# dropbox/rust-brotli

Measured on AMD Instinct MI355X. Metric: compress MB/s at q5 lgwin22, higher is better.
Workload: dtype u8; 1 GPU; 64 MiB synthetic English-like text per GPU, quality=5, lgwin=22, one-shot BrotliEncoderCompress (H6), input and stream resident in HBM; input_bytes_total=67108864, compressed_bytes=16370400

## Files before the change

### rust-brotli_amd/csrc/lz77_kernels.hip

```cpp
#include <hip/hip_runtime.h>
#include <stdexcept>
#include <string>
#include <utility>
#include <string.h>
#include <mutex>
#include <vector>

#include "device_api.h"
#include "lz77_chain.h"
#include "lz77_rows.h"
#include "lz77_groups.h"
#include "device_scan.h"
#include "lz77_parse_args.h"
#include "zopfli_device.h"
#include "batch_greedy_device.h"

namespace brotli_mi355x {

void hip_check(hipError_t e, const char* what) {
  if (e == hipSuccess) return;
  (void)hipGetLastError();
  throw std::runtime_error(std::string("HIP error in ") + what + ": " + hipGetErrorString(e));
}

__global__ __launch_bounds__(256) void k_compute_keys(const uint8_t* __restrict__ text, uint16_t* __restrict__ keys,
                                                      uint32_t n, uint32_t valid_n, uint32_t kind, uint32_t bucket_bits,
                                                      uint64_t hash_mask, uint32_t* __restrict__ run_samples,
                                                      const uint16_t* __restrict__ dict_hash, uint32_t* __restrict__ dict_items) {
  uint32_t i = blockIdx.x * blockDim.x + threadIdx.x;
  const uint32_t stride = gridDim.x * blockDim.x;
  for (; i < n; i += stride) {
    if (dict_items != nullptr) {
      const uint32_t h = ((br_load32(text + i) * 0x1e35a7bdu) >> (32 - 14)) << 1;
      dict_items[i] = (uint32_t)dict_hash[h] | ((uint32_t)dict_hash[h + 1] << 16);
    }
    uint32_t key = 0xffffu;
    if (i < valid_n) {
      if ((i & 63u) == 0 && i + 16 <= n) {
        const uint64_t v = br_load64(text + i);
        if (v == (v & 0xffull) * 0x0101010101010101ull && br_load64(text + i + 8) == v && *(volatile uint32_t*)run_samples < 4096u)
          atomicAdd(run_samples, 1u);
      }
      if (kind == 6) {
        const uint64_t v = (br_load64(text + i) & hash_mask) * 0x1fe35a7bd3579bd3ull;
        key = (uint32_t)(v >> (64 - bucket_bits));
      } else {
        const uint32_t v = br_load32(text + i) * 0x1e35a7bdu;
        key = v >> (32 - bucket_bits);
      }
    }
    keys[i] = (uint16_t)key;
  }
  if (dict_items != nullptr && blockIdx.x == 0 && threadIdx.x == 0) {
    const uint32_t h = ((br_load32(text + n) * 0x1e35a7bdu) >> (32 - 14)) << 1;
    dict_items[n] = (uint32_t)dict_hash[h] | ((uint32_t)dict_hash[h + 1] << 16);
  }
}

void lz77_compute_keys(const Lz77Params& P, const Lz77Buffers& B) {
  const uint32_t n = P.total_bytes;
  const uint32_t valid_n = n >= P.htl ? n - P.htl + 1 : 0;
  const uint64_t hash_mask = P.hasher_kind == 6 ? (0xffffffffffffffffull >> (64 - 8 * P.hash_len)) : 0;
  if (n == 0) return;
  uint32_t blocks = (n + 255) / 256;
  if (blocks > 8192) blocks = 8192;
  dev_memset(B.changed_count + 8, 0, 4);
  hipLaunchKernelGGL(k_compute_keys, dim3(blocks), dim3(256), 0, BR_STREAM, B.text, B.keys, n, valid_n, P.hasher_kind, P.bucket_bits,
                     hash_mask, B.changed_count + 8, dev_tables().dict_hash, B.dict_items);
  HIP_CHECK(hipGetLastError());
}

__global__ __launch_bounds__(64) void k_init_flag_tails(const Segment* __restrict__ segments, uint32_t num_segments, uint32_t htl,
                                                         uint8_t* __restrict__ flags) {
  const uint32_t k = blockIdx.x * blockDim.x + threadIdx.x;
  if (k >= num_segments) return;
  const Segment g = segments[k];
  if (!(g.flags & kSegFirstInBlock)) return;
  const uint32_t bs = g.blk_start, be = g.blk_end;
  if (g.block_index == 0 && be - bs >= htl - 1 && bs >= 3) flags[bs - 3] = flags[bs - 2] = flags[bs - 1] = 1;
  const uint32_t store_end = (be - bs >= htl) ? be - htl + 1 : bs;
  for (uint32_t q = store_end; q < be; ++q) flags[q] = (q + 3 >= be && (g.flags & kSegTailStitched)) ? 1 : 0;
}

void lz77_init_flags(const Lz77Params& P, const Lz77Buffers& B, uint32_t first_block_start, const uint8_t* prefix_flags_host,
                     uint32_t prefix_flags_bytes) {
  const uint32_t M = P.total_bytes, P0 = P.prefix_bytes, htl = P.htl;
  dev_memset(B.flags[0], 0, (size_t)M + 64);
  if (P0 > htl - 1) HIP_CHECK(hipMemsetAsync(B.flags[0], 1, P0 - (htl - 1), BR_STREAM));
  if (prefix_flags_host && prefix_flags_bytes) {
    HIP_CHECK(hipMemcpyAsync(B.flags[0], prefix_flags_host, prefix_flags_bytes, hipMemcpyHostToDevice, BR_STREAM));
  }
  if (M > first_block_start) HIP_CHECK(hipMemsetAsync(B.flags[0] + first_block_start, 1, M - first_block_start, BR_STREAM));
  if (P.num_segments) {
    hipLaunchKernelGGL(k_init_flag_tails, dim3((P.num_segments + 63) / 64), dim3(64), 0, BR_STREAM, B.segments, P.num_segments, htl, B.flags[0]);
  }
  HIP_CHECK(hipMemcpyAsync(B.flags[1], B.flags[0], (size_t)M + 64, hipMemcpyDeviceToDevice, BR_STREAM));
  HIP_CHECK(hipGetLastError());
}

static constexpr uint32_t kSortTile = 4096;

__global__ __launch_bounds__(256) void k_radix_hist(const uint16_t* __restrict__ keys, uint32_t n, uint32_t shift,
                                                     uint32_t num_tiles, uint32_t* __restrict__ hist) {
  __shared__ uint32_t h[256];
  h[threadIdx.x] = 0;
  __syncthreads();
  const uint32_t base = blockIdx.x * kSortTile;
  for (uint32_t r = 0; r < 16; ++r) {
    const uint32_t i = base + r * 256 + threadIdx.x;
    if (i < n) atomicAdd(&h[(keys[i] >> shift) & 255u], 1u);
  }
  __syncthreads();
  hist[threadIdx.x * num_tiles + blockIdx.x] = h[threadIdx.x];
}

__global__ __launch_bounds__(256) void k_radix_scatter(const uint16_t* __restrict__ keys_in, const uint32_t* __restrict__ vals_in,
                                                        uint16_t* __restrict__ keys_out, uint32_t* __restrict__ vals_out, uint32_t n,
                                                        uint32_t shift, uint32_t num_tiles, const uint32_t* __restrict__ offsets,
                                                        const uint8_t* __restrict__ text, const uint16_t* __restrict__ tags_in,
                                                        uint16_t* __restrict__ tags_out) {
  __shared__ uint32_t gbase[256];
  __shared__ uint32_t lstart[256];
  __shared__ uint32_t run[256];
  __shared__ uint32_t wcount[4][256];
  __shared__ uint32_t wave_total[4];
  __shared__ uint16_t skey[kSortTile];
  __shared__ uint32_t sval[kSortTile];
  __shared__ uint16_t stagv[kSortTile];
  const int tid = threadIdx.x, lane = tid & 63, w = tid >> 6;
  const uint32_t tile_base = blockIdx.x * kSortTile;
  const uint32_t tile_n = n - tile_base < kSortTile ? n - tile_base : kSortTile;
  {
    const uint32_t idx = (uint32_t)tid * num_tiles + blockIdx.x;
    const uint32_t here = offsets[idx];
    const uint32_t next = idx + 1 < 256u * num_tiles ? offsets[idx + 1] : n;
    const uint32_t count = next - here;
    gbase[tid] = here;
    uint32_t incl = count;
    for (uint32_t off = 1; off < 64; off <<= 1) {
      const uint32_t up = (uint32_t)__shfl_up((int)incl, off, 64);
      if ((uint32_t)lane >= off) incl += up;
    }
    if (lane == 63) wave_total[w] = incl;
    __syncthreads();
    uint32_t before = 0;
    for (int i = 0; i < w; ++i) before += wave_total[i];
    lstart[tid] = before + incl - count;
    run[tid] = before + incl - count;
  }
  __syncthreads();
  for (uint32_t r = 0; r < 16; ++r) {
    const uint32_t i = tile_base + r * 256 + tid;
    const bool valid = i < n;
    uint32_t key = 0, val = 0, d = 0, tag = 0;
    if (valid) {
      key = keys_in[i];
      val = vals_in ? vals_in[i] : i;
      d = (key >> shift) & 255u;
      if (tags_out) tag = tags_in ? tags_in[i] : br_tag16(br_load32(text + val));
    }
#pragma unroll
    for (int j = 0; j < 4; ++j) wcount[w][lane * 4 + j] = 0;
    __syncthreads();
    unsigned long long peers = __ballot(valid);
#pragma unroll
    for (int bit = 0; bit < 8; ++bit) {
      const bool one = (d >> bit) & 1u;
      const unsigned long long b = __ballot(one);
      peers &= one ? b : ~b;
    }
    const uint32_t rank_in_wave = __popcll(peers & ((1ull << lane) - 1ull));
    if (valid && rank_in_wave == 0) wcount[w][d] = __popcll(peers);
    __syncthreads();
    if (valid) {
      uint32_t at = run[d] + rank_in_wave;
      for (int i2 = 0; i2 < w; ++i2) at += wcount[i2][d];
      skey[at] = (uint16_t)key;
      sval[at] = val;
      if (tags_out) stagv[at] = (uint16_t)tag;
    }
    __syncthreads();
    run[tid] += wcount[0][tid] + wcount[1][tid] + wcount[2][tid] + wcount[3][tid];
    __syncthreads();
  }
  for (uint32_t at = tid; at < tile_n; at += 256) {
    const uint32_t key = skey[at];
    const uint32_t d = (key >> shift) & 255u;
    const uint32_t dst = gbase[d] + (at - lstart[d]);
    keys_out[dst] = (uint16_t)key;
    vals_out[dst] = sval[at];
    if (tags_out) tags_out[dst] = stagv[at];
  }
}

size_t lz77_sort_tmp_bytes(uint32_t total_bytes) {
  const size_t n = total_bytes;
  const size_t tiles = (n + kSortTile - 1) / kSortTile + 1;
  return n * 10 + 2048 + tiles * 256 * 4 + (tiles * 256 / kScanTile + 1024) * 8 + (n / kScanTile + 1024) * 8 + 4096;
}

void lz77_key_ranges(const Lz77Params& P, const Lz77Buffers& B);

void lz77_sort_by_key(const Lz77Params& P, const Lz77Buffers& B) {
  const uint32_t n = P.total_bytes;
  if (n == 0) return;
  const uint32_t tiles = (n + kSortTile - 1) / kSortTile;
  uint8_t* tmp = (uint8_t*)B.sort_tmp;
  uint16_t* keys_tmp = (uint16_t*)tmp;
  tmp += ((size_t)n * 2 + 255) & ~(size_t)255;
  uint32_t* vals_tmp = (uint32_t*)tmp;
  tmp += ((size_t)n * 4 + 255) & ~(size_t)255;
  uint16_t* tags_tmp = (uint16_t*)tmp;
  tmp += ((size_t)n * 2 + 255) & ~(size_t)255;
  uint32_t* hist = (uint32_t*)tmp;
  tmp += (size_t)tiles * 256 * 4;
  uint32_t* scratch = (uint32_t*)tmp;
  hipLaunchKernelGGL(k_radix_hist, dim3(tiles), dim3(256), 0, BR_STREAM, B.keys, n, 0u, tiles, hist);
  exclusive_scan_u32(hist, tiles * 256, scratch);
  hipLaunchKernelGGL(k_radix_scatter, dim3(tiles), dim3(256), 0, BR_STREAM, B.keys, (const uint32_t*)nullptr, keys_tmp, vals_tmp, n, 0u, tiles,
                     hist, (const uint8_t*)B.text, (const uint16_t*)nullptr, B.stag ? tags_tmp : (uint16_t*)nullptr);
  hipLaunchKernelGGL(k_radix_hist, dim3(tiles), dim3(256), 0, BR_STREAM, keys_tmp, n, 8u, tiles, hist);
  exclusive_scan_u32(hist, tiles * 256, scratch);
  hipLaunchKernelGGL(k_radix_scatter, dim3(tiles), dim3(256), 0, BR_STREAM, keys_tmp, vals_tmp, B.sorted_keys, B.by_key, n, 8u, tiles, hist,
                     (const uint8_t*)B.text, (const uint16_t*)tags_tmp, B.stag);
  HIP_CHECK(hipGetLastError());
  lz77_key_ranges(P, B);
}

__global__ __launch_bounds__(256) void k_key_ranges(const uint16_t* __restrict__ sorted_keys, uint32_t n, uint32_t* __restrict__ key_first,
                                                     uint32_t* __restrict__ key_last) {
  const uint32_t i = blockIdx.x * blockDim.x + threadIdx.x;
  if (i >= n) return;
  const uint16_t k = sorted_keys[i];
  if (i == 0 || sorted_keys[i - 1] != k) key_first[k] = i;
  if (i + 1 == n || sorted_keys[i + 1] != k) key_last[k] = i + 1;
}

struct InitialFlagGeometry {
  uint32_t enabled, first_block_start, prefix_bytes, block_bytes, total_bytes, prefix_stored_end;
};

__global__ __launch_bounds__(256) void k_rank_gather(const uint32_t* __restrict__ by_key, const uint8_t* __restrict__ flags, uint32_t n,
                                                      uint8_t* __restrict__ fbits, uint32_t* __restrict__ tile_sums,
                                                      InitialFlagGeometry ig, uint32_t masked_bits) {
  __shared__ uint32_t wave_sum[4];
  const uint32_t base = blockIdx.x * kScanTile + threadIdx.x * 4;
  uint32_t local = 0, packed = 0;
#pragma unroll
  for (int j = 0; j < 4; ++j)
    if (base + j < n) {
      const uint32_t p = by_key[base + j];
      uint32_t f;
      bool known = false;
      if (ig.enabled) {
        if (p >= ig.first_block_start) {
          known = ((p - ig.prefix_bytes) % ig.block_bytes) + 16 < ig.block_bytes && p + 16 < ig.total_bytes;
        } else {
          known = p + 16 < ig.prefix_stored_end;
        }
      }
      const uint32_t fl = known ? 1u : (uint32_t)flags[p];
      f = fl & 1u;
      packed |= (f | ((masked_bits && (fl & kFlagMasked)) ? kSlotMasked : 0u)) << (8 * j);
      local += f;
    }
  if (base < n) *(uint32_t*)(fbits + base) = packed;
  for (int off = 32; off > 0; off >>= 1) local += __shfl_down(local, off, 64);
  if ((threadIdx.x & 63) == 0) wave_sum[threadIdx.x >> 6] = local;
  __syncthreads();
  if (threadIdx.x == 0) tile_sums[blockIdx.x] = wave_sum[0] + wave_sum[1] + wave_sum[2] + wave_sum[3];
}

__global__ __launch_bounds__(256) void k_key_bases(const uint8_t* __restrict__ fbits, const uint32_t* __restrict__ tile_offsets,
                                                    const uint32_t* __restrict__ key_first, const uint32_t* __restrict__ key_last,
                                                    uint32_t* __restrict__ key_base) {
  const uint32_t k = blockIdx.x * blockDim.x + threadIdx.x;
  if (k >= 65536) return;
  const uint32_t i0 = key_first[k];
  if (key_last[k] <= i0) return;
  const uint32_t tile = i0 / kScanTile;
  uint32_t g = tile_offsets[tile];
  uint32_t i = tile * kScanTile;
  for (; i + 4 <= i0; i += 4) g += (*(const uint32_t*)(fbits + i) * 0x01010101u) >> 24;
  for (; i < i0; ++i) g += fbits[i];
  key_base[k] = g;
}

__device__ __forceinline__ uint32_t ring_count_at(uint32_t p, uint32_t local_rank, uint32_t key, const uint32_t* count_base, uint32_t reset_pos,
                                                  const uint32_t* reset_counts);
__device__ __forceinline__ uint32_t ring_count(uint32_t local_rank, uint32_t base) {
  const uint32_t num = (local_rank + base) & 0xffffu;
  return num < local_rank ? num : local_rank;
}

__device__ __forceinline__ uint32_t ring_count_at(uint32_t p, uint32_t local_rank, uint32_t key, const uint32_t* count_base, uint32_t reset_pos,
                                                  const uint32_t* reset_counts) {
  if (reset_pos != 0 && p >= reset_pos) {
    const uint32_t since = local_rank - reset_counts[key];
    return since & 0xffffu;
  }
  return ring_count(local_rank, count_base ? count_base[key] : 0u);
}

__global__ __launch_bounds__(256) void k_rank_apply(const uint32_t* __restrict__ by_key, const uint16_t* __restrict__ sorted_keys,
                                                     const uint8_t* __restrict__ fbits, uint32_t n, const uint32_t* __restrict__ tile_offsets,
                                                     const uint32_t* __restrict__ key_first, const uint32_t* __restrict__ key_base,
                                                     uint32_t* __restrict__ sorted, uint2* __restrict__ info,
                                                     const uint32_t* __restrict__ count_base, uint32_t reset_pos,
                                                     const uint32_t* __restrict__ reset_counts, const uint16_t* __restrict__ stag,
                                                     uint16_t* __restrict__ sorted_tag, const uint8_t* __restrict__ flags_if_masked) {
  __shared__ uint32_t wave_sum[4];
  const uint32_t base = blockIdx.x * kScanTile + threadIdx.x * 4;
  uint32_t pos[4], f[4], key[4];
  uint32_t local = 0;
  const uint32_t packed = base < n ? *(const uint32_t*)(fbits + base) : 0u;
#pragma unroll
  for (int j = 0; j < 4; ++j) {
    pos[j] = 0;
    key[j] = 0;
    f[j] = (packed >> (8 * j)) & 1u;
    if (base + j < n) {
      pos[j] = by_key[base + j];
      key[j] = sorted_keys[base + j];
    } else {
      f[j] = 0;
    }
    local += f[j];
  }
  uint32_t x = local;
  const int lane = threadIdx.x & 63, w = threadIdx.x >> 6;
#pragma unroll
  for (int off = 1; off < 64; off <<= 1) {
    uint32_t y = __shfl_up(x, off, 64);
    if (lane >= off) x += y;
  }
  if (lane == 63) wave_sum[w] = x;
  __syncthreads();
  uint32_t g = tile_offsets[blockIdx.x] + x - local;
  for (int i = 0; i < w; ++i) g += wave_sum[i];
#pragma unroll
  for (int j = 0; j < 4; ++j) {
    if (base + j < n) {
      const uint32_t lr = g - key_base[key[j]];
      const uint32_t slot = key_first[key[j]] + lr;
      info[pos[j]] = make_uint2(slot, ring_count_at(pos[j], lr, key[j], count_base, reset_pos, reset_counts));
      if (f[j]) {
        sorted[slot] = pos[j] | ((flags_if_masked != nullptr && (flags_if_masked[pos[j]] & kFlagMasked)) ? kMaskedEntry : 0u);
        if (sorted_tag) sorted_tag[slot] = stag[base + j];
      }
      g += f[j];
    }
  }
}

void lz77_key_ranges(const Lz77Params& P, const Lz77Buffers& B) {
  const uint32_t n = P.total_bytes;
  dev_memset(B.key_first, 0, 65537 * 4);
  dev_memset(B.key_last, 0, 65537 * 4);
  if (n == 0) return;
  hipLaunchKernelGGL(k_key_ranges, dim3((n + 255) / 256), dim3(256), 0, BR_STREAM, B.sorted_keys, n, B.key_first, B.key_last);
  HIP_CHECK(hipGetLastError());
}

void lz77_rank_flags(const Lz77Params& P, const Lz77Buffers& B, int which, int rbuf, const RankInitialHint* initial) {
  const uint32_t n = P.total_bytes;
  if (n == 0) return;
  InitialFlagGeometry ig{};
  if (initial) {
    ig.enabled = 1;
    ig.first_block_start = initial->first_block_start;
    ig.prefix_bytes = P.prefix_bytes;
    ig.block_bytes = initial->block_bytes;
    ig.total_bytes = n;
    ig.prefix_stored_end = (initial->prefix_is_dictionary && P.prefix_bytes > P.htl - 1) ? P.prefix_bytes - (P.htl - 1) : 0;
  }
  const uint32_t tiles = (n + kScanTile - 1) / kScanTile;
  uint32_t* tile_sums = (uint32_t*)B.sort_tmp;
  uint32_t* scratch = tile_sums + tiles + 64;
  if (P.reset_pos) lz77_key_counts(P, B, which, P.reset_vis, B.reset_counts, false);
  hipLaunchKernelGGL(k_rank_gather, dim3(tiles), dim3(256), 0, BR_STREAM, B.by_key, B.flags[which], n, B.fbits, tile_sums, ig, 0u);
  exclusive_scan_u32(tile_sums, tiles, scratch);
  hipLaunchKernelGGL(k_key_bases, dim3(256), dim3(256), 0, BR_STREAM, B.fbits, tile_sums, B.key_first, B.key_last, B.key_base);
  hipLaunchKernelGGL(k_rank_apply, dim3(tiles), dim3(256), 0, BR_STREAM, B.by_key, B.sorted_keys, B.fbits, n, tile_sums, B.key_first, B.key_base,
                     B.sorted[rbuf], (uint2*)B.info[rbuf], B.count_base, P.reset_pos, B.reset_counts, B.stag, B.stag ? B.sorted_tag[rbuf] : nullptr,
                     P.masked_from != kNeverMasked ? (const uint8_t*)B.flags[which] : (const uint8_t*)nullptr);
  HIP_CHECK(hipGetLastError());
}

__device__ __forceinline__ void note_rows_changed(uint32_t k, uint32_t p, uint32_t* rows_lo, uint32_t* rows_hi) {
  if (rows_lo == nullptr) return;
  atomicMin(&rows_lo[k], p);
  atomicMax(&rows_hi[k], p);
}
__device__ __forceinline__ void mark_dirty(uint32_t p, const SegGeometry& geo, uint8_t* __restrict__ dirty, uint32_t* rows_lo = nullptr,
                                           uint32_t* rows_hi = nullptr) {
  const uint32_t blk = (p - geo.prefix_bytes) / geo.block_bytes;
  const uint32_t bs = blk == 0 ? geo.first_block_start : geo.prefix_bytes + blk * geo.block_bytes;
  const uint32_t off = p - bs;
  const uint32_t seg_bytes = geo.block_segment_bytes[blk];
  uint32_t k = geo.block_first_segment[blk] + off / seg_bytes;
  if (k >= geo.block_first_segment[blk + 1]) k = geo.block_first_segment[blk + 1] - 1;
  dirty[k] = 1;
  note_rows_changed(k, p, rows_lo, rows_hi);
  if (k > 0 && (off % seg_bytes) < 8) {
    dirty[k - 1] = 1;
    note_rows_changed(k - 1, p, rows_lo, rows_hi);
  }
}

__device__ __forceinline__ uint32_t chain_in_front_if_near_boundary(uint32_t p, const SegGeometry& geo) {
  const uint32_t blk = (p - geo.prefix_bytes) / geo.block_bytes;
  const uint32_t bs = blk == 0 ? geo.first_block_start : geo.prefix_bytes + blk * geo.block_bytes;
  const uint32_t off = p - bs;
  const uint32_t seg_bytes = geo.block_segment_bytes[blk];
  const uint32_t first = geo.block_first_segment[blk];
  uint32_t k = first + off / seg_bytes;
  if (k >= geo.block_first_segment[blk + 1]) return 0xffffffffu;
  if (k == first || (off % seg_bytes) >= 8) return 0xffffffffu;
  return k - 1;
}

__device__ __forceinline__ uint32_t block_sum_256(uint32_t v, uint32_t* wave_sum) {
  for (int off = 32; off > 0; off >>= 1) v += __shfl_down(v, off, 64);
  __syncthreads();
  if ((threadIdx.x & 63) == 0) wave_sum[threadIdx.x >> 6] = v;
  __syncthreads();
  return wave_sum[0] + wave_sum[1] + wave_sum[2] + wave_sum[3];
}

__global__ __launch_bounds__(256) void k_rerank_count(const RerankChunk* __restrict__ chunks, const uint32_t* __restrict__ by_key,
                                                       const uint8_t* __restrict__ flags, uint32_t* __restrict__ sums) {
  __shared__ uint32_t wave_sum[4];
  const RerankChunk c = chunks[blockIdx.x];
  uint32_t local = 0;
  for (uint32_t i = c.begin + threadIdx.x; i < c.end; i += 256) local += flags[by_key[i]] & 1u;
  const uint32_t total = block_sum_256(local, wave_sum);
  if (threadIdx.x == 0) sums[c.my_sum] = total;
}

__global__ __launch_bounds__(256) void k_rerank_apply(const RerankChunk* __restrict__ chunks, const uint32_t* __restrict__ sums,
                                                       const uint32_t* __restrict__ by_key, const uint8_t* __restrict__ flags,
                                                       uint32_t* __restrict__ rank_tmp, uint32_t* __restrict__ sorted_tmp) {
  __shared__ uint32_t wave_sum[4];
  __shared__ uint32_t running;
  const RerankChunk c = chunks[blockIdx.x];
  const int lane = threadIdx.x & 63, w = threadIdx.x >> 6;
  uint32_t before = 0;
  for (uint32_t j = c.first_sum + threadIdx.x; j < c.my_sum; j += 256) before += sums[j];
  before = block_sum_256(before, wave_sum);
  if (threadIdx.x == 0) running = before;
  __syncthreads();
  for (uint32_t tile = c.begin; tile < c.end; tile += kScanTile) {
    const uint32_t base = tile + threadIdx.x * 4;
    uint32_t pos[4], f[4], masked[4], local = 0;
#pragma unroll
    for (int j = 0; j < 4; ++j) {
      pos[j] = 0;
      f[j] = 0;
      masked[j] = 0;
      if (base + j < c.end) {
        pos[j] = by_key[base + j];
        const uint32_t fl = flags[pos[j]];
        f[j] = fl & 1u;
        masked[j] = (fl & kFlagMasked) ? kMaskedEntry : 0u;
      }
      local += f[j];
    }
    uint32_t x = local;
#pragma unroll
    for (int off = 1; off < 64; off <<= 1) {
      uint32_t y = __shfl_up(x, off, 64);
      if (lane >= off) x += y;
    }
    if (lane == 63) wave_sum[w] = x;
    __syncthreads();
    uint32_t g = running + x - local;
    for (int i = 0; i < w; ++i) g += wave_sum[i];
#pragma unroll
    for (int j = 0; j < 4; ++j) {
      if (base + j < c.end) {
        rank_tmp[base + j] = g;
        if (f[j]) sorted_tmp[c.key_lo + g] = pos[j] | masked[j];
        g += f[j];
      }
    }
    __syncthreads();
    if (threadIdx.x == 0) running += wave_sum[0] + wave_sum[1] + wave_sum[2] + wave_sum[3];
    __syncthreads();
  }
}

__device__ __forceinline__ void list_or_mark(uint32_t p, const SegGeometry& geo, uint8_t* dirty, uint32_t* recheck_list, uint32_t* recheck_count,
                                             uint32_t recheck_cap) {
  if (recheck_list != nullptr) {
    const uint32_t at = atomicAdd(recheck_count, 1u);
    if (at < recheck_cap) {
      recheck_list[at] = p;
      return;
    }
  }
  mark_dirty(p, geo, dirty);
}

__global__ __launch_bounds__(256) void k_rerank_check(const uint8_t* __restrict__ text, const RerankChunk* __restrict__ chunks,
                                                       const uint32_t* __restrict__ by_key,
                                                       const uint8_t* __restrict__ flags, const uint32_t* __restrict__ sorted,
                                                       const uint2* __restrict__ info, const uint32_t* __restrict__ rank_tmp,
                                                       const uint32_t* __restrict__ sorted_tmp, SegGeometry geo,
                                                       uint8_t* __restrict__ dirty, const uint32_t* __restrict__ count_base,
                                                       const uint16_t* __restrict__ keys, uint32_t reset_pos,
                                                       const uint32_t* __restrict__ reset_counts, uint32_t* __restrict__ recheck_list,
                                                       uint32_t* __restrict__ recheck_count, uint32_t recheck_cap) {
  const RerankChunk c = chunks[blockIdx.x];
  for (uint32_t i = c.begin + threadIdx.x; i < c.end; i += 256) {
// ... 2221 lines not shown
```

### rust-brotli_amd/csrc/lz77_stage.cpp

```cpp
#include "lz77_stage.h"
#include "timeline.h"

#include <math.h>
#include <stdio.h>
#include <stdlib.h>
#include <string.h>

#include <algorithm>
#include <chrono>
#include <map>
#include <stdexcept>
#include <string>

#include "host_entropy.h"

#include <cmath>

namespace brotli_mi355x {

void Lz77Stage::Release() {
  mem_.clear();
  L_ = LiveBuffers{};
  Z_ = ZopfliJob{};
  S_ = QuickSpec{};
// ... 2190 lines not shown
      for (uint32_t k = 0; k < nseg; ++k) {
        n_dirty_valid += cand_dirty[k];
        dirty[k] |= cand_dirty[k];
      }
      tm.stop(&stats_.ms_rank);
      stamp("dirty-here");
    }
    const bool regime_flip = dict_death_seg_ != 0xffffffffu && dict_death_seg_ != last_death_seg && dict_flips_ > 64;
    for (uint32_t k = 0; k < nseg; ++k) entry_streak[k] = dirty_entry_[k] ? (uint8_t)std::min<uint32_t>(entry_streak[k] + 1u, 255u) : (uint8_t)0;
    if (const char* first = getenv("BROTLI_MI355X_DEBUG_MAP")) {
      const uint32_t a = std::max<uint32_t>((uint32_t)atoi(first), 0u) ? (uint32_t)atoi(first) : 16u;
      std::string m;
      for (uint32_t k = a; k < a + 32 && k < nseg; ++k) m += dirty_entry_[k] ? (pending[k] ? 'P' : 'E') : (dirty[k] ? 'c' : '.');
      fprintf(stderr, "  map[%u..%u) %s\n", a, a + 32, m.c_str());
      for (uint32_t k = a; k < a + 12 && k < nseg; ++k)
        fprintf(stderr, "    seg %u [%u,%u) used pos %u apply %u head %u/%u cache %d %d %d %d | chained pos %u apply %u head %u/%u cache %d %d %d %d | exit pos %u cmds %u searches %u\n",
                k, segments_[k].start, segments_[k].end, entries_[k].pos, entries_[k].apply, entries_[k].head_kind, entries_[k].head_base,
                entries_[k].cache[0], entries_[k].cache[1], entries_[k].cache[2], entries_[k].cache[3], next_entries_[k].pos,
                next_entries_[k].apply, next_entries_[k].head_kind, next_entries_[k].head_base, next_entries_[k].cache[0],
                next_entries_[k].cache[1], next_entries_[k].cache[2], next_entries_[k].cache[3], exits_[k].pos, exits_[k].n_cmds,
                exits_[k].n_searches);
    }
    if (const char* path = getenv("BROTLI_MI355X_DEBUG_DIRTY")) {
      if (FILE* f = fopen(path, "a")) {
        std::string m(nseg, '.');
        for (uint32_t k = 0; k < nseg; ++k) {
          const bool c = !cand_dirty.empty() && cand_dirty[k];
          m[k] = dirty_entry_[k] ? (c ? 'B' : (pending[k] ? 'P' : 'E')) : (c ? 'c' : (dirty[k] ? 'p' : '.'));
        }
        std::string why(nseg, '0');
        for (uint32_t k = 0; k < nseg; ++k) why[k] = (char)('0' + (entry_reason_[k] & 3));
        fprintf(f, "%s %s\n", m.c_str(), why.c_str());
        fclose(f);
      }
    }
    was_dirty = dirty;
    const bool aggressive = false;
    count = 0;
    bool front_run = false;
    cache_wave_next.assign(nseg, 0);
    for (uint32_t k = 0; k < nseg; ++k) {
      sched[k] = 0;
      if (segments_[k].flags & kSegFirstInBlock) front_run = false;
      if (!dirty[k]) {
        front_run = false;
        continue;
      }
      const bool must_redo = pending[k] || (!cand_dirty.empty() && cand_dirty[k]);
      if (front_run && !dirty_entry_[k]) {
        sched[k] = 2;
        pending[k] = 1;
        dirty[k] = 0;
        continue;
      }
      front_run = false;
      const bool passes_cache_along = entry_reason_[k] == 2 && exits_[k].n_cmds == 0 && exits_[k].ext_len == 0 &&
                                      getenv("BROTLI_MI355X_DEFER_CACHE_ONLY") == nullptr;
      const bool defer = (aggressive || entry_streak[k] >= 2) && !(segments_[k].flags & kSegFirstInBlock) && k > 0 && was_dirty[k - 1] &&
                         !predicted_entry_[k] && !passes_cache_along;
      if (defer) {
        sched[k] = must_redo ? 2 : 0;
        pending[k] = must_redo;
        dirty[k] = 0;
        continue;
      }
      sched[k] = (dirty_entry_[k] || pending[k]) ? kSchedOwn : kSchedOwnRows;
      pending[k] = 0;
      list[count++] = k;
      entries_[k] = next_entries_[k];
      TouchSegment(k);
      const bool cache_only = dirty_entry_[k] && entry_reason_[k] == 2;
      cache_wave_next[k] = cache_only;
      front_run = follow_cache_fronts && cache_only && k > 0 && !(segments_[k].flags & kSegFirstInBlock) && cache_wave[k - 1];
    }
    cache_wave.swap(cache_wave_next);
    if (regime_flip) {
      last_death_seg = dict_death_seg_;
      static const bool no_regime_warmup = getenv("BROTLI_MI355X_NO_REGIME_WARMUP") != nullptr;
      if (warmup_bytes_ > 0 && dict_death_seg_ + 2 < nseg && !no_regime_warmup) {
        Warmup(dict_death_seg_ + 1, true, which, rbuf, &dirty);
        for (uint32_t k = dict_death_seg_ + 1; k < nseg; ++k)
          if (sched[k] == kSchedOwnRows) sched[k] = kSchedOwn;
      }
    }
    if (getenv("BROTLI_MI355X_DEBUG")) fprintf(stderr, "mismatch pos %u apply %u cache %u apply-only %u | block-first: cache %u ext %u | head %u; dict death seg %u (forecast %u) flips %u\n", dbg_counts_[0], dbg_counts_[1], dbg_counts_[2], dbg_counts_[3], dbg_first_[0], dbg_first_[1], dbg_first_[2], dict_death_seg_, predicted_death_, dict_flips_);
    if (getenv("BROTLI_MI355X_DEBUG")) fprintf(stderr, "  resolver: %u of %u blocks taken over from the last pass\n", resolve_blocks_skipped_, (unsigned)block_segment_bytes_.size());
    if (getenv("BROTLI_MI355X_DEBUG")) fprintf(stderr, "round %u: flag changes %llu, dirty segments %u of %u (entry %u, candidates %u), predicted literal runs %u, cache rechecks passed %u\n", round, (unsigned long long)n_changed, count, nseg, n_dirty_entry, n_dirty_valid, predicted_runs_, rechecked);
    host_schedule_ms_ += std::chrono::duration<double, std::milli>(std::chrono::steady_clock::now() - host_t1).count();
    stamp("scheduled");
    if (count == 0) {
      if (const char* path = getenv("BROTLI_MI355X_DEBUG_FRONT")) {
        if (FILE* f = fopen(path, "a")) {
          fprintf(f, "FINAL");
          for (uint32_t k = 0; k < nseg; ++k) fprintf(f, " %u:%u", exits_[k].pos, exits_[k].n_cmds);
          fprintf(f, "\n");
          fclose(f);
        }
      }
      done = true;
      break;
    }
    full_round = false;
  }
  resolve_incremental_ = false;
  tmp.clear();
  if (restart) {
    saved_block_guess_.clear();
    for (uint32_t k = 0; k < nseg; ++k)
      if (segments_[k].flags & kSegFirstInBlock) saved_block_guess_[segments_[k].blk_start] = next_entries_[k];
    Resegment(segment_bytes_);
    stats_.coarse_restarts++;
    RunRounds(false);
    return;
  }
  if (!done) throw std::runtime_error("brotli_mi355x: backward-reference search did not reach a fixed point");
  final_flags_ = which;
  if (selftest) {
    if (use_rows_) SelfTestRows(which); else SelfTestRank(which, rbuf);
  }
  tm.stop(&stats_.ms_resolve);
  if (getenv("BROTLI_MI355X_DEBUG_EXITS"))
    for (uint32_t k = 0; k < nseg && k < 40; ++k)
      fprintf(stderr, "  seg %u [%u,%u) entry pos %u | exit pos %u insert %u cmds %u lits %u searches %u\n", k, segments_[k].start, segments_[k].end,
              entries_[k].pos, exits_[k].pos, exits_[k].insert_len, exits_[k].n_cmds, exits_[k].n_lits, exits_[k].n_searches);
  for (uint32_t k = 0; k < nseg; ++k) stats_.searches += exits_[k].n_searches;
}


void Lz77Stage::DumpFlags(uint8_t* out, size_t size) const {
  dev_sync();
  dev_d2h(out, B_.flags[final_flags_], std::min<size_t>(size, P_.total_bytes));
}

void Lz77Stage::SelfTestSort() {
  const uint32_t n = P_.total_bytes;
  std::vector<uint16_t> keys(n), skeys(n);
  std::vector<uint32_t> by_key(n);
  dev_sync();
  dev_d2h(keys.data(), B_.keys, (size_t)n * 2);
  dev_d2h(skeys.data(), B_.sorted_keys, (size_t)n * 2);
  dev_d2h(by_key.data(), B_.by_key, (size_t)n * 4);
  std::vector<uint8_t> seen(n, 0);
  for (uint32_t i = 0; i < n; ++i) {
    const uint32_t p = by_key[i];
    if (p >= n || seen[p]) throw std::runtime_error("selftest: by_key is not a permutation at slot " + std::to_string(i));
    seen[p] = 1;
    if (skeys[i] != keys[p]) throw std::runtime_error("selftest: sorted_keys mismatch at slot " + std::to_string(i));
    if (i > 0) {
      if (skeys[i - 1] > skeys[i]) throw std::runtime_error("selftest: keys not ascending at slot " + std::to_string(i));
      if (skeys[i - 1] == skeys[i] && by_key[i - 1] >= p)
        throw std::runtime_error("selftest: sort not stable at slot " + std::to_string(i));
    }
  }
}

void Lz77Stage::SelfTestRank(int which, int rbuf) {
  const uint32_t n = P_.total_bytes;
  std::vector<uint16_t> skeys(n);
  std::vector<uint32_t> by_key(n), sorted(n), info((size_t)n * 2);
  std::vector<uint8_t> flags(n);
  dev_sync();
  dev_d2h(skeys.data(), B_.sorted_keys, (size_t)n * 2);
  dev_d2h(by_key.data(), B_.by_key, (size_t)n * 4);
  dev_d2h(sorted.data(), B_.sorted[rbuf], (size_t)n * 4);
  dev_d2h(info.data(), B_.info[rbuf], (size_t)n * 8);
  dev_d2h(flags.data(), B_.flags[which], n);
  uint32_t first = 0, local = 0;
  for (uint32_t i = 0; i < n; ++i) {
    const uint32_t p = by_key[i];
    if (i == 0 || skeys[i - 1] != skeys[i]) {
      first = i;
      local = 0;
      if (key_first_[skeys[i]] != i) throw std::runtime_error("selftest: key_first mismatch for key " + std::to_string(skeys[i]));
    }
    if (i + 1 == n || skeys[i + 1] != skeys[i]) {
      if (key_last_[skeys[i]] != i + 1) throw std::runtime_error("selftest: key_last mismatch for key " + std::to_string(skeys[i]));
    }
    const bool plain_counters = B_.count_base == nullptr && P_.reset_pos == 0;
    const uint32_t visible = std::min(local & 0xffffu, local);
    if (info[2 * (size_t)p] != first + local || (plain_counters && info[2 * (size_t)p + 1] != visible))
      throw std::runtime_error("selftest: info mismatch at slot " + std::to_string(i));
    if (flags[p] & 1) {
      if (sorted[first + local] != p) throw std::runtime_error("selftest: sorted mismatch at slot " + std::to_string(i));
      local++;
    }
  }
}

void Lz77Stage::SelfTestRows(int which) {
  const uint32_t n = P_.total_bytes;
  std::vector<uint16_t> skeys(n);
  std::vector<uint32_t> by_key(n), rows((size_t)n * kRowEntries);
  std::vector<uint8_t> flags(n), fbits(n), text((size_t)n + 64, 0);
  dev_sync();
  dev_d2h(skeys.data(), B_.sorted_keys, (size_t)n * 2);
  dev_d2h(by_key.data(), B_.by_key, (size_t)n * 4);
  dev_d2h(rows.data(), B_.rows, (size_t)n * kRowEntries * 4);
  dev_d2h(flags.data(), B_.flags[which], n);
  dev_d2h(fbits.data(), B_.fbits, n);
  dev_d2h(text.data(), B_.text, n);
  auto tag = [&](uint32_t p) {
    uint32_t v;
    memcpy(&v, text.data() + p, 4);
    return (uint32_t)((v * 0x9E3779B1u) >> 16);
  };
  const uint32_t depth = 1u << P_.block_bits;
  uint32_t first = 0, stored_before = 0, local_before = 0, since_reset = 0;
  for (uint32_t i = 0; i < n; ++i) {
    const uint32_t p = by_key[i];
    if (i == 0 || skeys[i - 1] != skeys[i]) {
      first = i;
      stored_before = B_.count_base ? carry_->key_counts[skeys[i]] : 0u;
      local_before = 0;
      since_reset = 0;
    }
    const uint32_t counter = (P_.reset_pos != 0 && p >= P_.reset_pos) ? since_reset : stored_before;
    if ((fbits[i] & 1) != (flags[p] & 1)) throw std::runtime_error("selftest: fbits mismatch at slot " + std::to_string(i));
    if (fbits[i] & 2) throw std::runtime_error("selftest: leftover change mark at slot " + std::to_string(i));
    {
      const bool big = P_.reset_pos != 0 || B_.count_base != nullptr || key_last_[skeys[i]] - key_first_[skeys[i]] >= 65536u;
      const bool want_wrap = big && counter != 0 && (counter & 0xffffu) == 0;
      if (want_wrap != ((fbits[i] & 4) != 0)) throw std::runtime_error("selftest: wrap mark mismatch at slot " + std::to_string(i));
    }
    const uint32_t max_backward = std::min(p, P_.max_backward_limit);
    const uint32_t d = std::min(depth, counter & 0xffffu);
    const uint32_t oldest = p >= P_.reset_pos ? P_.reset_vis : 0u;
    std::vector<uint32_t> want;
    uint32_t seen = 0;
    for (uint32_t j = i; j > first && seen < d;) {
      --j;
      if (!(flags[by_key[j]] & 1)) continue;
      if (p - by_key[j] > max_backward || by_key[j] < oldest) break;
      ++seen;
      if (tag(by_key[j]) == tag(p)) want.push_back(by_key[j]);
    }
    for (size_t c = 0; c <= want.size() && c < kRowEntries; ++c) {
      const uint32_t have = rows[(size_t)p * kRowEntries + c];
      const uint32_t expect = c < want.size() ? want[c] : kRowEnd;
      if (have != expect)
        throw std::runtime_error("selftest: row of position " + std::to_string(p) + " entry " + std::to_string(c) + ": " + std::to_string(have) +
                                 " instead of " + std::to_string(expect));
    }
    stored_before += flags[p] & 1;
    local_before += flags[p] & 1;
    if (P_.reset_pos != 0 && p >= P_.reset_vis) since_reset += flags[p] & 1;
  }
  (void)local_before;
}

void Lz77Stage::KeyCountsBetween(uint32_t from, uint32_t upto, std::vector<uint32_t>* out) {
  DevBlocks tmp;
  uint32_t* dev = tmp.zeroed<uint32_t>(2 * 65536 * 4);
  lz77_key_counts(P_, B_, final_flags_, upto, dev, false);
  lz77_key_counts(P_, B_, final_flags_, from, dev + 65536, false);
  std::vector<uint32_t> both(2 * 65536);
  dev_d2h(both.data(), dev, both.size() * 4);
  tmp.clear();
  out->resize(65536);
  for (uint32_t k = 0; k < 65536; ++k) (*out)[k] = both[k] - both[65536 + k];
}

void Lz77Stage::KeyCountsBefore(uint32_t upto, std::vector<uint32_t>* out) {
  DevBlocks tmp;
  uint32_t* dev = tmp.zeroed<uint32_t>(65536 * 4);
  lz77_key_counts(P_, B_, final_flags_, upto, dev);
  out->resize(65536);
  dev_d2h(out->data(), dev, 65536 * 4);
}

void Lz77Stage::Gather() {
  const uint32_t nseg = (uint32_t)segments_.size();
  for (uint32_t k = 0; k < nseg; ++k)
    if (exits_[k].bad_commands != 0)
      throw std::runtime_error(
          "brotli_mi355x: the reference encoder fails on this input: a match cut to one byte at the end of the custom dictionary "
          "gives a copy it cannot encode (fix_unbroken_len, backward_references/mod.rs:42-54; GetCopyLengthCode, command.rs:91-93)");
  std::vector<uint32_t> offsets(nseg), counts(nseg);
  std::vector<CmdPatch> fix, fix_ext;
  size_t t = 0, ti = 0;
  uint64_t total = 0;
  for (uint32_t k = 0; k < nseg; ++k) {
    offsets[k] = (uint32_t)total;
    counts[k] = exits_[k].n_cmds;
    total += exits_[k].n_cmds;
    while (ti < trailing_.size() && trailing_[ti].after_segment == k) {
      CmdPatch p{};
      p.index = (uint32_t)total;
      p.kind = 1;
      p.value = trailing_[ti].insert_len;
      fix.push_back(p);
      total++;
      ti++;
    }
  }
  (void)t;
  for (const Carry& c : carries_) {
    CmdPatch p{};
    p.index = offsets[c.segment];
    p.kind = 2;
    p.value = c.literals;
    fix.push_back(p);
  }
  for (const Patch& pt : patches_) {
    CmdPatch p{};
    p.index = offsets[pt.segment] + pt.index;
    p.kind = 0;
// ... 30 lines not shown
```

Before: 4288 MB/s.

## Fuse radix sort histogram and key-range pass into neighbouring kernels

The first-pass radix histogram now comes out of the key-computation kernel, which walks the input in sort tiles and counts keys in shared memory. That removes a separate histogram launch and a re-read of the keys. The scatter kernel is rewritten to hold 16 elements per thread in registers, rank them per wave with ballots and wave barriers instead of block-wide syncs on every round, and is templated on the first pass. The final scatter also writes key_first/key_last with atomics, replacing the separate key-range kernel at the cost of an extra fix-up launch. The sort now depends on the histogram having been produced earlier by the key kernel, which couples the two stages.

```diff
diff --git a/rust-brotli_amd/csrc/lz77_kernels.hip b/rust-brotli_amd/csrc/lz77_kernels.hip
--- a/rust-brotli_amd/csrc/lz77_kernels.hip
+++ b/rust-brotli_amd/csrc/lz77_kernels.hip
@@ -23,38 +23,78 @@
   throw std::runtime_error(std::string("HIP error in ") + what + ": " + hipGetErrorString(e));
 }
 
+static constexpr uint32_t kSortTile = 4096;
+
 __global__ __launch_bounds__(256) void k_compute_keys(const uint8_t* __restrict__ text, uint16_t* __restrict__ keys,
                                                       uint32_t n, uint32_t valid_n, uint32_t kind, uint32_t bucket_bits,
                                                       uint64_t hash_mask, uint32_t* __restrict__ run_samples,
-                                                      const uint16_t* __restrict__ dict_hash, uint32_t* __restrict__ dict_items) {
-  uint32_t i = blockIdx.x * blockDim.x + threadIdx.x;
-  const uint32_t stride = gridDim.x * blockDim.x;
-  for (; i < n; i += stride) {
-    if (dict_items != nullptr) {
-      const uint32_t h = ((br_load32(text + i) * 0x1e35a7bdu) >> (32 - 14)) << 1;
-      dict_items[i] = (uint32_t)dict_hash[h] | ((uint32_t)dict_hash[h + 1] << 16);
-    }
-    uint32_t key = 0xffffu;
-    if (i < valid_n) {
-      if ((i & 63u) == 0 && i + 16 <= n) {
-        const uint64_t v = br_load64(text + i);
-        if (v == (v & 0xffull) * 0x0101010101010101ull && br_load64(text + i + 8) == v && *(volatile uint32_t*)run_samples < 4096u)
-          atomicAdd(run_samples, 1u);
+                                                      const uint16_t* __restrict__ dict_hash, uint32_t* __restrict__ dict_items,
+                                                      uint32_t num_tiles, uint32_t* __restrict__ hist) {
+  __shared__ uint32_t h[256];
+  for (uint32_t tile = blockIdx.x; tile < num_tiles; tile += gridDim.x) {
+    const uint32_t tile_base = tile * kSortTile;
+    const uint32_t tile_n = n - tile_base < kSortTile ? n - tile_base : kSortTile;
+    if (hist != nullptr) {
+      h[threadIdx.x] = 0;
+      __syncthreads();
+    }
+#pragma unroll 4
+    for (uint32_t e = threadIdx.x; e < tile_n; e += 256) {
+      const uint32_t i = tile_base + e;
+      if (dict_items != nullptr) {
+        const uint32_t dh = ((br_load32(text + i) * 0x1e35a7bdu) >> (32 - 14)) << 1;
+        dict_items[i] = (uint32_t)dict_hash[dh] | ((uint32_t)dict_hash[dh + 1] << 16);
       }
-      if (kind == 6) {
-        const uint64_t v = (br_load64(text + i) & hash_mask) * 0x1fe35a7bd3579bd3ull;
-        key = (uint32_t)(v >> (64 - bucket_bits));
-      } else {
-        const uint32_t v = br_load32(text + i) * 0x1e35a7bdu;
-        key = v >> (32 - bucket_bits);
+      uint32_t key = 0xffffu;
+      if (i < valid_n) {
+        if ((i & 63u) == 0 && i + 16 <= n) {
+          const uint64_t v = br_load64(text + i);
+          if (v == (v & 0xffull) * 0x0101010101010101ull && br_load64(text + i + 8) == v && *(volatile uint32_t*)run_samples < 4096u)
+            atomicAdd(run_samples, 1u);
+        }
+        if (kind == 6) {
+          const uint64_t v = (br_load64(text + i) & hash_mask) * 0x1fe35a7bd3579bd3ull;
+          key = (uint32_t)(v >> (64 - bucket_bits));
+        } else {
+          const uint32_t v = br_load32(text + i) * 0x1e35a7bdu;
+          key = v >> (32 - bucket_bits);
+        }
       }
-    }
-    keys[i] = (uint16_t)key;
+      keys[i] = (uint16_t)key;
+      if (hist != nullptr) atomicAdd(&h[key & 255u], 1u);
+    }
+    if (hist != nullptr) {
+      __syncthreads();
+      hist[threadIdx.x * num_tiles + tile] = h[threadIdx.x];
+    }
   }
   if (dict_items != nullptr && blockIdx.x == 0 && threadIdx.x == 0) {
-    const uint32_t h = ((br_load32(text + n) * 0x1e35a7bdu) >> (32 - 14)) << 1;
-    dict_items[n] = (uint32_t)dict_hash[h] | ((uint32_t)dict_hash[h + 1] << 16);
-  }
+    const uint32_t dh = ((br_load32(text + n) * 0x1e35a7bdu) >> (32 - 14)) << 1;
+    dict_items[n] = (uint32_t)dict_hash[dh] | ((uint32_t)dict_hash[dh + 1] << 16);
+  }
+}
+
+struct SortScratch {
+  uint16_t* keys_tmp;
+  uint32_t* vals_tmp;
+  uint16_t* tags_tmp;
+  uint32_t* hist;
+  uint32_t* scratch;
+};
+static SortScratch sort_scratch(const Lz77Buffers& B, uint32_t n) {
+  const uint32_t tiles = (n + kSortTile - 1) / kSortTile;
+  SortScratch s;
+  uint8_t* tmp = (uint8_t*)B.sort_tmp;
+  s.keys_tmp = (uint16_t*)tmp;
+  tmp += ((size_t)n * 2 + 255) & ~(size_t)255;
+  s.vals_tmp = (uint32_t*)tmp;
+  tmp += ((size_t)n * 4 + 255) & ~(size_t)255;
+  s.tags_tmp = (uint16_t*)tmp;
+  tmp += ((size_t)n * 2 + 255) & ~(size_t)255;
+  s.hist = (uint32_t*)tmp;
+  tmp += (size_t)tiles * 256 * 4;
+  s.scratch = (uint32_t*)tmp;
+  return s;
 }
 
 void lz77_compute_keys(const Lz77Params& P, const Lz77Buffers& B) {
@@ -62,11 +102,11 @@
   const uint32_t valid_n = n >= P.htl ? n - P.htl + 1 : 0;
   const uint64_t hash_mask = P.hasher_kind == 6 ? (0xffffffffffffffffull >> (64 - 8 * P.hash_len)) : 0;
   if (n == 0) return;
-  uint32_t blocks = (n + 255) / 256;
-  if (blocks > 8192) blocks = 8192;
+  const uint32_t tiles = (n + kSortTile - 1) / kSortTile;
+  uint32_t* hist = (B.sort_tmp != nullptr && B.sort_tmp_bytes >= lz77_sort_tmp_bytes(n)) ? sort_scratch(B, n).hist : nullptr;
   dev_memset(B.changed_count + 8, 0, 4);
-  hipLaunchKernelGGL(k_compute_keys, dim3(blocks), dim3(256), 0, BR_STREAM, B.text, B.keys, n, valid_n, P.hasher_kind, P.bucket_bits,
-                     hash_mask, B.changed_count + 8, dev_tables().dict_hash, B.dict_items);
+  hipLaunchKernelGGL(k_compute_keys, dim3(tiles < 8192 ? tiles : 8192), dim3(256), 0, BR_STREAM, B.text, B.keys, n, valid_n, P.hasher_kind,
+                     P.bucket_bits, hash_mask, B.changed_count + 8, dev_tables().dict_hash, B.dict_items, tiles, hist);
   HIP_CHECK(hipGetLastError());
 }
 
@@ -98,8 +138,6 @@
   HIP_CHECK(hipGetLastError());
 }
 
-static constexpr uint32_t kSortTile = 4096;
-
 __global__ __launch_bounds__(256) void k_radix_hist(const uint16_t* __restrict__ keys, uint32_t n, uint32_t shift,
                                                      uint32_t num_tiles, uint32_t* __restrict__ hist) {
   __shared__ uint32_t h[256];
@@ -114,15 +152,16 @@
   hist[threadIdx.x * num_tiles + blockIdx.x] = h[threadIdx.x];
 }
 
-__global__ __launch_bounds__(256) void k_radix_scatter(const uint16_t* __restrict__ keys_in, const uint32_t* __restrict__ vals_in,
+template <bool kFirstPass>
+__global__ __launch_bounds__(256) __attribute__((amdgpu_waves_per_eu(4, 4))) void k_radix_scatter(const uint16_t* __restrict__ keys_in, const uint32_t* __restrict__ vals_in,
                                                         uint16_t* __restrict__ keys_out, uint32_t* __restrict__ vals_out, uint32_t n,
                                                         uint32_t shift, uint32_t num_tiles, const uint32_t* __restrict__ offsets,
                                                         const uint8_t* __restrict__ text, const uint16_t* __restrict__ tags_in,
-                                                        uint16_t* __restrict__ tags_out) {
+                                                        uint16_t* __restrict__ tags_out, uint32_t* __restrict__ key_first,
+                                                        uint32_t* __restrict__ key_last) {
   __shared__ uint32_t gbase[256];
-  __shared__ uint32_t lstart[256];
-  __shared__ uint32_t run[256];
-  __shared__ uint32_t wcount[4][256];
+  __shared__ uint32_t lstart[257];
+  __shared__ uint32_t wbase[4][256];
   __shared__ uint32_t wave_total[4];
   __shared__ uint16_t skey[kSortTile];
   __shared__ uint32_t sval[kSortTile];
@@ -130,38 +169,54 @@
   const int tid = threadIdx.x, lane = tid & 63, w = tid >> 6;
   const uint32_t tile_base = blockIdx.x * kSortTile;
   const uint32_t tile_n = n - tile_base < kSortTile ? n - tile_base : kSortTile;
+  const uint32_t hidx = (uint32_t)tid * num_tiles + blockIdx.x;
+  const uint32_t here = offsets[hidx];
+  const uint32_t next = hidx + 1 < 256u * num_tiles ? offsets[hidx + 1] : n;
+  uint32_t key[16], val[16], tag[16];
+  const uint32_t e0 = (uint32_t)w * 1024u + (uint32_t)lane;
+#pragma unroll
+  for (int r = 0; r < 16; ++r) {
+    const uint32_t e = e0 + (uint32_t)r * 64u;
+    key[r] = keys_in[tile_base + (e < tile_n ? e : tile_n - 1)];
+  }
+#pragma unroll
+  for (int r = 0; r < 16; ++r) {
+    const uint32_t e = e0 + (uint32_t)r * 64u;
+    const uint32_t i = tile_base + (e < tile_n ? e : tile_n - 1);
+    val[r] = kFirstPass ? i : vals_in[i];
+  }
+  if (tags_out != nullptr) {
+#pragma unroll
+    for (int r = 0; r < 16; ++r) {
+      const uint32_t e = e0 + (uint32_t)r * 64u;
+      const uint32_t i = tile_base + (e < tile_n ? e : tile_n - 1);
+      tag[r] = kFirstPass ? br_tag16(br_load32(text + i)) : (uint32_t)tags_in[i];
+    }
+  }
+  const uint32_t count = next - here;
+  uint32_t start;
   {
-    const uint32_t idx = (uint32_t)tid * num_tiles + blockIdx.x;
-    const uint32_t here = offsets[idx];
-    const uint32_t next = idx + 1 < 256u * num_tiles ? offsets[idx + 1] : n;
-    const uint32_t count = next - here;
     gbase[tid] = here;
     uint32_t incl = count;
-    for (uint32_t off = 1; off < 64; off <<= 1) {
-      const uint32_t up = (uint32_t)__shfl_up((int)incl, off, 64);
-      if ((uint32_t)lane >= off) incl += up;
+    for (uint32_t o = 1; o < 64; o <<= 1) {
+      const uint32_t up = (uint32_t)__shfl_up((int)incl, o, 64);
+      if ((uint32_t)lane >= o) incl += up;
     }
     if (lane == 63) wave_total[w] = incl;
+#pragma unroll
+    for (int j = 0; j < 4; ++j) wbase[w][lane * 4 + j] = 0;
     __syncthreads();
     uint32_t before = 0;
     for (int i = 0; i < w; ++i) before += wave_total[i];
-    lstart[tid] = before + incl - count;
-    run[tid] = before + incl - count;
-  }
-  __syncthreads();
-  for (uint32_t r = 0; r < 16; ++r) {
-    const uint32_t i = tile_base + r * 256 + tid;
-    const bool valid = i < n;
-    uint32_t key = 0, val = 0, d = 0, tag = 0;
-    if (valid) {
-      key = keys_in[i];
-      val = vals_in ? vals_in[i] : i;
-      d = (key >> shift) & 255u;
-      if (tags_out) tag = tags_in ? tags_in[i] : br_tag16(br_load32(text + val));
-    }
-#pragma unroll
-    for (int j = 0; j < 4; ++j) wcount[w][lane * 4 + j] = 0;
-    __syncthreads();
+    start = before + incl - count;
+    lstart[tid] = start;
+    if (tid == 255) lstart[256] = start + count;
+  }
+  volatile uint32_t* mine = wbase[w];
+#pragma unroll
+  for (int r = 0; r < 16; ++r) {
+    const bool valid = e0 + (uint32_t)r * 64u < tile_n;
+    const uint32_t d = (key[r] >> shift) & 255u;
     unsigned long long peers = __ballot(valid);
 #pragma unroll
     for (int bit = 0; bit < 8; ++bit) {
@@ -170,27 +225,49 @@
       peers &= one ? b : ~b;
     }
     const uint32_t rank_in_wave = __popcll(peers & ((1ull << lane) - 1ull));
-    if (valid && rank_in_wave == 0) wcount[w][d] = __popcll(peers);
-    __syncthreads();
-    if (valid) {
-      uint32_t at = run[d] + rank_in_wave;
-      for (int i2 = 0; i2 < w; ++i2) at += wcount[i2][d];
-      skey[at] = (uint16_t)key;
-      sval[at] = val;
-      if (tags_out) stagv[at] = (uint16_t)tag;
-    }
-    __syncthreads();
-    run[tid] += wcount[0][tid] + wcount[1][tid] + wcount[2][tid] + wcount[3][tid];
-    __syncthreads();
-  }
+    const uint32_t seen = mine[d];
+    key[r] |= (seen + rank_in_wave) << 16;
+    __builtin_amdgcn_wave_barrier();
+    if (valid && rank_in_wave == 0) mine[d] = seen + (uint32_t)__popcll(peers);
+    __builtin_amdgcn_wave_barrier();
+  }
+  __syncthreads();
+  {
+    const uint32_t c0 = wbase[0][tid], c1 = wbase[1][tid], c2 = wbase[2][tid];
+    wbase[0][tid] = start;
+    wbase[1][tid] = start + c0;
+    wbase[2][tid] = start + c0 + c1;
+    wbase[3][tid] = start + c0 + c1 + c2;
+  }
+  __syncthreads();
+#pragma unroll
+  for (int r = 0; r < 16; ++r) {
+    if (e0 + (uint32_t)r * 64u < tile_n) {
+      const uint32_t at = wbase[w][(key[r] >> shift) & 255u] + (key[r] >> 16);
+      skey[at] = (uint16_t)key[r];
+      sval[at] = val[r];
+      if (tags_out != nullptr) stagv[at] = (uint16_t)tag[r];
+    }
+  }
+  __syncthreads();
   for (uint32_t at = tid; at < tile_n; at += 256) {
-    const uint32_t key = skey[at];
-    const uint32_t d = (key >> shift) & 255u;
-    const uint32_t dst = gbase[d] + (at - lstart[d]);
-    keys_out[dst] = (uint16_t)key;
+    const uint32_t k = skey[at];
+    const uint32_t d = (k >> shift) & 255u;
+    const uint32_t ls = lstart[d];
+    const uint32_t dst = gbase[d] + (at - ls);
+    keys_out[dst] = (uint16_t)k;
     vals_out[dst] = sval[at];
-    if (tags_out) tags_out[dst] = stagv[at];
-  }
+    if (tags_out != nullptr) tags_out[dst] = stagv[at];
+    if (!kFirstPass && key_first != nullptr) {
+      if (at == ls || skey[at - 1] != k) atomicMin(&key_first[k], dst);
+      if (at + 1 == lstart[d + 1] || skey[at + 1] != k) atomicMax(&key_last[k], dst + 1);
+    }
+  }
+}
+
+__global__ __launch_bounds__(256) void k_key_first_absent(uint32_t* __restrict__ key_first) {
+  const uint32_t k = blockIdx.x * blockDim.x + threadIdx.x;
+  if (k < 65537 && key_first[k] == 0xffffffffu) key_first[k] = 0;
 }
 
 size_t lz77_sort_tmp_bytes(uint32_t total_bytes) {
@@ -199,41 +276,24 @@
   return n * 10 + 2048 + tiles * 256 * 4 + (tiles * 256 / kScanTile + 1024) * 8 + (n / kScanTile + 1024) * 8 + 4096;
 }
 
-void lz77_key_ranges(const Lz77Params& P, const Lz77Buffers& B);
-
 void lz77_sort_by_key(const Lz77Params& P, const Lz77Buffers& B) {
   const uint32_t n = P.total_bytes;
   if (n == 0) return;
+  if (B.sort_tmp == nullptr || B.sort_tmp_bytes < lz77_sort_tmp_bytes(n)) throw std::runtime_error("brotli_mi355x: key sort without its scratch");
   const uint32_t tiles = (n + kSortTile - 1) / kSortTile;
-  uint8_t* tmp = (uint8_t*)B.sort_tmp;
-  uint16_t* keys_tmp = (uint16_t*)tmp;
-  tmp += ((size_t)n * 2 + 255) & ~(size_t)255;
-  uint32_t* vals_tmp = (uint32_t*)tmp;
-  tmp += ((size_t)n * 4 + 255) & ~(size_t)255;
-  uint16_t* tags_tmp = (uint16_t*)tmp;
-  tmp += ((size_t)n * 2 + 255) & ~(size_t)255;
-  uint32_t* hist = (uint32_t*)tmp;
-  tmp += (size_t)tiles * 256 * 4;
-  uint32_t* scratch = (uint32_t*)tmp;
-  hipLaunchKernelGGL(k_radix_hist, dim3(tiles), dim3(256), 0, BR_STREAM, B.keys, n, 0u, tiles, hist);
-  exclusive_scan_u32(hist, tiles * 256, scratch);
-  hipLaunchKernelGGL(k_radix_scatter, dim3(tiles), dim3(256), 0, BR_STREAM, B.keys, (const uint32_t*)nullptr, keys_tmp, vals_tmp, n, 0u, tiles,
-                     hist, (const uint8_t*)B.text, (const uint16_t*)nullptr, B.stag ? tags_tmp : (uint16_t*)nullptr);
-  hipLaunchKernelGGL(k_radix_hist, dim3(tiles), dim3(256), 0, BR_STREAM, keys_tmp, n, 8u, tiles, hist);
-  exclusive_scan_u32(hist, tiles * 256, scratch);
-  hipLaunchKernelGGL(k_radix_scatter, dim3(tiles), dim3(256), 0, BR_STREAM, keys_tmp, vals_tmp, B.sorted_keys, B.by_key, n, 8u, tiles, hist,
-                     (const uint8_t*)B.text, (const uint16_t*)tags_tmp, B.stag);
-  HIP_CHECK(hipGetLastError());
-  lz77_key_ranges(P, B);
-}
-
-__global__ __launch_bounds__(256) void k_key_ranges(const uint16_t* __restrict__ sorted_keys, uint32_t n, uint32_t* __restrict__ key_first,
-                                                     uint32_t* __restrict__ key_last) {
-  const uint32_t i = blockIdx.x * blockDim.x + threadIdx.x;
-  if (i >= n) return;
-  const uint16_t k = sorted_keys[i];
-  if (i == 0 || sorted_keys[i - 1] != k) key_first[k] = i;
-  if (i + 1 == n || sorted_keys[i + 1] != k) key_last[k] = i + 1;
+  const SortScratch s = sort_scratch(B, n);
+  HIP_CHECK(hipMemsetAsync(B.key_first, 0xff, 65537 * 4, BR_STREAM));
+  dev_memset(B.key_last, 0, 65537 * 4);
+  exclusive_scan_u32(s.hist, tiles * 256, s.scratch);
+  hipLaunchKernelGGL(k_radix_scatter<true>, dim3(tiles), dim3(256), 0, BR_STREAM, B.keys, (const uint32_t*)nullptr, s.keys_tmp, s.vals_tmp, n, 0u,
+                     tiles, s.hist, (const uint8_t*)B.text, (const uint16_t*)nullptr, B.stag ? s.tags_tmp : (uint16_t*)nullptr,
+                     (uint32_t*)nullptr, (uint32_t*)nullptr);
+  hipLaunchKernelGGL(k_radix_hist, dim3(tiles), dim3(256), 0, BR_STREAM, s.keys_tmp, n, 8u, tiles, s.hist);
+  exclusive_scan_u32(s.hist, tiles * 256, s.scratch);
+  hipLaunchKernelGGL(k_radix_scatter<false>, dim3(tiles), dim3(256), 0, BR_STREAM, s.keys_tmp, s.vals_tmp, B.sorted_keys, B.by_key, n, 8u, tiles,
+                     s.hist, (const uint8_t*)B.text, (const uint16_t*)s.tags_tmp, B.stag, B.key_first, B.key_last);
+  hipLaunchKernelGGL(k_key_first_absent, dim3((65537 + 255) / 256), dim3(256), 0, BR_STREAM, B.key_first);
+  HIP_CHECK(hipGetLastError());
 }
 
 struct InitialFlagGeometry {
@@ -351,15 +411,6 @@
       g += f[j];
     }
   }
-}
-
-void lz77_key_ranges(const Lz77Params& P, const Lz77Buffers& B) {
-  const uint32_t n = P.total_bytes;
-  dev_memset(B.key_first, 0, 65537 * 4);
-  dev_memset(B.key_last, 0, 65537 * 4);
-  if (n == 0) return;
-  hipLaunchKernelGGL(k_key_ranges, dim3((n + 255) / 256), dim3(256), 0, BR_STREAM, B.sorted_keys, n, B.key_first, B.key_last);
-  HIP_CHECK(hipGetLastError());
 }
 
 void lz77_rank_flags(const Lz77Params& P, const Lz77Buffers& B, int which, int rbuf, const RankInitialHint* initial) {
diff --git a/rust-brotli_amd/csrc/lz77_stage.cpp b/rust-brotli_amd/csrc/lz77_stage.cpp
--- a/rust-brotli_amd/csrc/lz77_stage.cpp
+++ b/rust-brotli_amd/csrc/lz77_stage.cpp
@@ -2366,6 +2366,27 @@
         throw std::runtime_error("selftest: sort not stable at slot " + std::to_string(i));
     }
   }
+  if (B_.stag) {
+    std::vector<uint16_t> stag(n);
+    std::vector<uint8_t> text((size_t)n + 64, 0);
+    dev_d2h(stag.data(), B_.stag, (size_t)n * 2);
+    dev_d2h(text.data(), B_.text, (size_t)n + 64);
+    for (uint32_t i = 0; i < n; ++i) {
+      uint32_t v;
+      memcpy(&v, text.data() + by_key[i], 4);
+      if (stag[i] != (uint16_t)((v * 0x9E3779B1u) >> 16)) throw std::runtime_error("selftest: stag mismatch at slot " + std::to_string(i));
+    }
+  }
+  std::vector<uint32_t> first(65537), last(65537), want_first(65537, 0), want_last(65537, 0);
+  dev_d2h(first.data(), B_.key_first, 65537 * 4);
+  dev_d2h(last.data(), B_.key_last, 65537 * 4);
+  for (uint32_t i = 0; i < n; ++i) {
+    if (i == 0 || skeys[i - 1] != skeys[i]) want_first[skeys[i]] = i;
+    if (i + 1 == n || skeys[i + 1] != skeys[i]) want_last[skeys[i]] = i + 1;
+  }
+  for (uint32_t k = 0; k < 65537; ++k)
+    if (first[k] != want_first[k] || last[k] != want_last[k])
+      throw std::runtime_error("selftest: key_first / key_last mismatch for key " + std::to_string(k));
 }
 
 void Lz77Stage::SelfTestRank(int which, int rbuf) {
```

Measured after the change: 4442 MB/s, median of 6. 3.6% higher.
